# rlglab/minizero

Hardware: AMD Instinct MI355X
Metric: self-play leaf-evals/s (9x9 Go AlphaZero n=400) (higher is better)
Workload: dtype f32; 1 GPU; BASELINE configs[1]: 9x9 Go AlphaZero, n=400, 6 blocks x 64 ch, 256 parallel games per GPU, synthetic fixed-weight net (seed 0), Dirichlet noise + random rotation + softmax-count moves (reference defaults); games_per_gpu=256, actor_num_simulation=400, pipeline_lanes=1, backend=nccl

## Files before the change

minizero_amd/csrc/net_body.h:

```cpp
#pragma once
#include "net_dev.h"
#include <type_traits>

#ifndef MZ_HPROF
#define MZ_HPROF(k)
#endif

namespace mz {

struct TowerArgs {
    int nlayers, cin0, C, OT;
    int in_bits;
    int has_stem;
    unsigned w_off[48], b_off[48];
};

template <int H, int W>
struct TileMap {
    static constexpr int P = H * W, PW = W + 2;
    static constexpr int PT = (P + 15) / 16;
    static constexpr bool kCorner = (P % 16 == 1) && H > 1 && W > 1 && PT >= 2;
    static constexpr int VQ = kCorner ? W - 1 : -1;
    static constexpr int PT0 = (PT + 1) / 2, PT1 = PT - PT0;
    short q[PT * 16];
// ... 493 lines not shown
        const float acc = (FP && xlds && xpw != 0) ? dotChain<16, true, true>(xrd + xo, xstride, w, 1, C) : dotChain<16>(xrd + xo, xstride, w, 1, C);
        float v = acc + ((j < PC) ? hp.pconv_b[j] : hp.vconv_b[0]);
        v = v > 0.0f ? v : 0.0f;
        if (j < PC) { pf[i] = v; } else { vf[p] = v; }
    }
    __syncthreads();
    MZ_HPROF(6);

    for (int a = tid; a < A; a += NT) {
        const float v = (BIGA ? dotChain<64, true, true>(pf, 1, hp.pfc_wT + a, A, PC * P) : FP ? dotChain<16, true, true>(pf, 1, hp.pfc_wT + a, A, PC * P) : dotChain<16>(pf, 1, hp.pfc_wT + a, A, PC * P)) + hp.pfc_b[a];
        lg[a] = v;
        logit[size_t(b) * A + a] = v;
    }
    if (BIGA && NT == 512 && A <= 384) {
        if (tid >= 384) {
            for (int o = tid - 384; o < VH; o += 256) {
                const int o2 = o + 128 < VH ? o + 128 : o;
                const float* const xs2[2] = {vf, vf};
                const float* const ws2[2] = {hp.vfc1_wT + o, hp.vfc1_wT + o2};
                float acc2[2];
                dotChainK<32, 2, true, true>(xs2, 1, ws2, VH, P, acc2);
                const float v0 = acc2[0] + hp.vfc1_b[o], v1 = acc2[1] + hp.vfc1_b[o2];
                h1[o] = v0 > 0.0f ? v0 : 0.0f;
                if (o + 128 < VH) { h1[o2] = v1 > 0.0f ? v1 : 0.0f; }
            }
        }
    } else {
        const int vo = (NT >= 256 && A <= 128) ? 128 : 0;
        for (int o = (tid - vo + NT) % NT; o < VH; o += NT) {
            const float v = (FP ? dotChain<16, true, true>(vf, 1, hp.vfc1_wT + o, VH, P) : dotChain<16>(vf, 1, hp.vfc1_wT + o, VH, P)) + hp.vfc1_b[o];
            h1[o] = v > 0.0f ? v : 0.0f;
        }
    }
    __syncthreads();
    MZ_HPROF(7);

    if (tid == 64) {
        const float acc = BIGA ? dotChain<32, true, true>(h1, 1, hp.vfc2_w, 1, VH) : FP ? dotChain<16, true, true>(h1, 1, hp.vfc2_w, 1, VH) : dotChain<16>(h1, 1, hp.vfc2_w, 1, VH);
        value[b] = mz_tanhf(acc + hp.vfc2_b[0]);
    }
    if (wave == 0) {
        float m = -3.4e38f;
        for (int a = lane; a < A; a += 64) { m = lg[a] > m ? lg[a] : m; }
        for (int o = 32; o > 0; o >>= 1) { float m2 = __shfl_xor(m, o); m = m2 > m ? m2 : m; }
        for (int a = lane; a < A; a += 64) { lg[a] = mz_expf(lg[a] - m); }
        __builtin_amdgcn_wave_barrier();
        __builtin_amdgcn_fence(__ATOMIC_ACQ_REL, "wavefront");
        const float s = orderedSumWave(lg, A, lane);
        for (int a = lane; a < A; a += 64) { policy[size_t(b) * A + a] = lg[a] / s; }
        MZ_HPROF(8);
    }
}


}
```

minizero_amd/csrc/sim.hip:

```cpp
#include "sim_az_body.h"
#include "sim_mz_body.h"

namespace mz {

MZ_SPEC_WAYS_IS(16);

template <int H, int W, int CIN0_PAD, int CDYN_PAD, int CPAD>
__global__ __launch_bounds__(512) void sim_kernel_mz(const SimArgs* __restrict__ a_, int sim0, int nsims, int host_start, int pre_epoch)
{
    CSimArgs* a = (CSimArgs*)a_;
    extern __shared__ __attribute__((aligned(16))) float tiles[];
    const int g = blockIdx.x, tid = threadIdx.x, lane = tid & 63, wave = tid >> 6;
    constexpr int CM = CIN0_PAD > CDYN_PAD ? (CIN0_PAD > CPAD ? CIN0_PAD : CPAD) : (CDYN_PAD > CPAD ? CDYN_PAD : CPAD);
    constexpr int kTileFloats = kTowerTiles * CM * planeStride(H, W);
    double* rcp_w = reinterpret_cast<double*>(tiles + kTileFloats);
    const int rcp_n = a->rcp_n;
    for (int i = tid; i < rcp_n; i += 512) { rcp_w[i] = a->pv.rcp_tab[i]; }
    LdsCDouble* rcp_lds = (LdsCDouble*)rcp_w;
    const int tab_n = rcp_n - 2;
    double* sqrt_w = rcp_w + rcp_n;
    float* bias_w = reinterpret_cast<float*>(sqrt_w + tab_n);
    int* spec_w = reinterpret_cast<int*>(bias_w + tab_n + (tab_n & 1));
    for (int i = tid; i < tab_n; i += 512) { sqrt_w[i] = a->pv.sqrt_tab[i]; bias_w[i] = a->pv.bias_tab[i]; }
    if (!a->atari) {
// ... 455 lines not shown
#ifdef MZ_SIM_TPROF
    {
        unsigned long long h[64];
        if (hipMemcpyFromSymbol(h, HIP_SYMBOL(g_tp), sizeof(h)) == hipSuccess && h[63]) {
            fprintf(stderr, "[mz sim tprof] cycles per layer (game 0, avg over %llu towers):", h[63]);
            for (int i = 0; i < 14; ++i) { fprintf(stderr, " %.0f", double(h[i]) / double(h[63])); }
            fprintf(stderr, "\n");
        }
    }
#endif
    if (sim_prof_.n == 0) { return; }
    hipLaunchKernelGGL(sim_prof_fold, dim3(1), dim3(1), 0, stream_, sim_prof_.p + sim_prof_.n - kSimProfTail);
    if (hipStreamSynchronize(stream_) != hipSuccess) { return; }
    std::vector<unsigned long long> h(sim_prof_.n);
    if (hipMemcpy(h.data(), sim_prof_.p, h.size() * sizeof(unsigned long long), hipMemcpyDeviceToHost) != hipSuccess) { return; }
    const std::vector<unsigned long long> tail(h.end() - kSimProfTail, h.end());
    h.resize(h.size() - kSimProfTail);
    double skipped = 0, skipped_max = 0, sims_all = 0;
    for (size_t g = 0; g < h.size() / 8; ++g) {
        const double sk = double(h[g * 8 + 4] >> 32);
        h[g * 8 + 4] &= 0xFFFFFFFFull;
        skipped += sk; sims_all += double(h[g * 8 + 4]);
        skipped_max = std::max(skipped_max, sk / std::max(1.0, double(h[g * 8 + 4])));
    }
    { double ps = 0, ac = 0, kk = 0; for (size_t g = 0; g < h.size() / 8; ++g) { ps += double(h[g * 8 + 7] >> 40); ac += double((h[g * 8 + 7] >> 20) & 0xFFFFF); kk += double(h[g * 8 + 7] & 0xFFFFF); } fprintf(stderr, "[mz sim prof] path speculation: %.0f passes, %.0f levels taken, %.0f walks that found a remembered path\n", ps, ac, kk); }
    const char* names[4] = {"select+leaf", "tower", "heads", "cand+expand"};
    const size_t G = h.size() / 8;
    double tot_all = 0, tot_max = 0;
    for (int k = 0; k < 4; ++k) {
        double sum = 0, mx = 0, sims = 0;
        for (size_t g = 0; g < G; ++g) { sum += double(h[g * 8 + k]); mx = std::max(mx, double(h[g * 8 + k])); sims += double(h[g * 8 + 4]); }
        fprintf(stderr, "[mz sim prof] %-12s avg %8.2f us per simulation (slowest game %8.2f us)\n", names[k], sum / std::max(1.0, sims) * 0.01,
                mx / std::max(1.0, sims / G) * 0.01);
        tot_all += sum / std::max(1.0, sims) * 0.01;
    }
    {
        double sel = 0, lev = 0, sims = 0, maxlev = 0;
        double helped = 0;
        const unsigned long long low = (1ull << 40) - 1;
        for (size_t g = 0; g < G; ++g) { sel += double(h[g * 8 + 5]); lev += double(h[g * 8 + 6] & low); helped += double(h[g * 8 + 6] >> 40); sims += double(h[g * 8 + 4]); maxlev = std::max(maxlev, double(h[g * 8 + 6] & low) / std::max(1.0, double(h[g * 8 + 4]))); }
        fprintf(stderr, "[mz sim prof] levels taken over from the helper waves: %.0f (%.1f %% of all levels)\n", helped, 100.0 * helped / std::max(1.0, lev));
        fprintf(stderr, "[mz sim prof] select alone avg %8.2f us, path length avg %.2f (deepest game avg %.2f) -> %.2f us per level\n", sel / std::max(1.0, sims) * 0.01,
                lev / std::max(1.0, sims), maxlev, sel / std::max(1.0, lev) * 0.01);
    }
    for (size_t g = 0; g < G; ++g) { tot_max = std::max(tot_max, double(h[g * 8] + h[g * 8 + 1] + h[g * 8 + 2] + h[g * 8 + 3]) / std::max(1.0, double(h[g * 8 + 4])) * 0.01); }
    fprintf(stderr, "[mz sim prof] total        avg %8.2f us per simulation (slowest game %8.2f us)\n", tot_all, tot_max);
    {
        double tw = 0, hd = 0;
        for (size_t g = 0; g < G; ++g) { tw += double(h[g * 8 + 1]); hd += double(h[g * 8 + 2]); }
        const double ran = std::max(1.0, sims_all - skipped);
        fprintf(stderr, "[mz sim prof] terminal leaves: network skipped in %.0f of %.0f simulations (%.2f %%; the game with the most: %.2f %%) -> per simulation that ran them: tower %.2f us, heads %.2f us\n",
                skipped, sims_all, 100.0 * skipped / std::max(1.0, sims_all), 100.0 * skipped_max, tw / ran * 0.01, hd / ran * 0.01);
    }
    fprintf(stderr, "[mz sim prof] value first: %llu of %.0f simulations in the new order; %llu walks arrived at the previous simulation's leaf, %llu waited there (avg %.2f us); "
                    "%llu waits at the join in front of the leaf\n",
            tail[16], sims_all, tail[17], tail[18], double(tail[19]) / std::max(1.0, double(tail[18])) * 0.01, tail[20]);
    if (tail[8] > 0) {
        const double L = double(tail[8]), first = double(tail[9]) / L * 0.01, last = double(tail[10]) / L * 0.01, mean = double(tail[11]) / L * 0.01;
        const double helping = double(tail[12]) / L * 0.01;
        fprintf(stderr, "[mz sim prof] launches: %llu, avg per launch from the first game's start: first game done %.1f us, mean %.1f us, last %.1f us -> %.1f %% of the CU time idles at the end of a launch\n",
                tail[8], first, mean, last, 100.0 * (last - mean - helping) / std::max(1e-9, last));
        if (tail[13] > 0 || tail[15] > 0 || tail[21] > 0) {
            double tw = 0;
            for (size_t g = 0; g < G; ++g) { tw += double(h[g * 8 + 1]); }
            const double ran = sims_all - skipped, qn = double(tail[21]), qt = double(tail[22]), pn = double(tail[13]) + qn, pt = double(tail[14]) + qt;
            const double ln = double(tail[33]), lt = double(tail[34]);
            fprintf(stderr, "[mz sim prof] tail help: %.0f of the %.0f simulations that ran the network had a pair tower (%.2f %%): tower %.2f us with a helper, %.2f us alone; %llu games helped, "
                            "a CU helps for %.1f us per launch after its own game (%.1f %% of the launch)\n",
                    pn, ran, 100.0 * pn / std::max(1.0, ran), pt / std::max(1.0, pn) * 0.01, (tw - pt - lt) / std::max(1.0, ran - pn - ln) * 0.01, tail[15], helping,
                    100.0 * helping / std::max(1e-9, last));
            fprintf(stderr, "[mz sim prof] tail help, quad towers: %.0f of the %.0f simulations that ran the network had a quad tower (%.2f %%): tower %.2f us with three helpers, %.2f us with "
                            "one; %llu games went from pair to quad towers\n",
                    qn, ran, 100.0 * qn / std::max(1.0, ran), qt / std::max(1.0, qn) * 0.01, (pt - qt) / std::max(1.0, pn - qn) * 0.01, tail[23]);
            const double ia = double(tail[30]) / L * 0.01, ib = double(tail[31]) / L * 0.01, ic = double(tail[32]) / L * 0.01;
            fprintf(stderr, "[mz sim prof] tail help, idle CU time by the reason the CU stopped looking for a game to help (%% of the launch): (a) every running game of its XCD had its "
                            "helpers %.2f %%, (b) no game of its XCD was running any more %.2f %%, (c) only games with fewer than help_min_left simulations were left %.2f %%\n",
                    100.0 * ia / std::max(1e-9, last), 100.0 * ib / std::max(1e-9, last), 100.0 * ic / std::max(1e-9, last));
        }
        if (tail[33] > 0 || tail[35] > 0 || tail[36] > 0) {
            const double ran = sims_all - skipped, ln = double(tail[33]), taken = double(tail[35]);
            fprintf(stderr, "[mz sim prof] lending: %.0f of the %.0f simulations that ran the network had a tower lent by a game that was ahead (%.2f %%): tower %.2f us with the volunteer; "
                            "%llu offers taken, %llu of them withdrawn behind a terminal leaf, %llu taken too late; a volunteer waits %.2f us for its command and is away for %.2f us per "
                            "offer taken, %.1f us per launch and CU (%.1f %% of the launch)\n",
                    ln, ran, 100.0 * ln / std::max(1.0, ran), double(tail[34]) / std::max(1.0, ln) * 0.01, tail[35], tail[37], tail[36], double(tail[38]) / std::max(1.0, taken) * 0.01,
                    double(tail[39]) / std::max(1.0, taken) * 0.01, double(tail[39]) / std::max(1.0, double(G)) / L * 0.01, 100.0 * double(tail[39]) / std::max(1.0, double(G)) / L * 0.01 / std::max(1e-9, last));
        }
    }
}

static size_t simLdsBound(size_t tile_bytes, int n, int A, size_t head_floats)
{
    const size_t rcp_n = size_t(n) + 5, max_depth = size_t(n) + 3;
    return tile_bytes + rcp_n * (2 * sizeof(double) + sizeof(float)) + kSpecWords * sizeof(int) + (size_t(5) * (A + 1) + 26 + 18 * 12 + 2 * max_depth + 2 + head_floats) * sizeof(float) +
           size_t(kGoSeenCap) * sizeof(uint64_t);
}

int Net::uploadSimArgs(const SimArgs& a)
{
    static_assert(sizeof(SimArgs) % 4 == 0, "SimArgs is copied as words");
    if (sim_args_host_.size() != sizeof(SimArgs) || memcmp(sim_args_host_.data(), &a, sizeof(SimArgs)) != 0) {
        if (!sim_args_.ensure(sizeof(SimArgs))) { setError("hipMalloc of the simulation arguments failed"); return MZ_ERR_DEVICE; }
        MZ_HIP(hipStreamSynchronize(stream_));
        MZ_HIP(hipMemcpy(sim_args_.p, &a, sizeof(SimArgs), hipMemcpyHostToDevice));
        sim_args_host_.assign(reinterpret_cast<const char*>(&a), reinterpret_cast<const char*>(&a) + sizeof(SimArgs));
    }
    return MZ_OK;
// ... 64 lines not shown
    a.use_gumbel = gum ? 1 : 0;
    if (gum) { a.gum = *gum; }
    a.start = d_start;
    a.no_spec = getenv("MZ_NO_SPEC") ? atoi(getenv("MZ_NO_SPEC")) : 0;
    if (getenv("MZ_SIM_PROF")) {
        rc = simProfBuffer(gv.games, &a.prof);
        if (rc) { return rc; }
    }
    if (wide) {
        if (precision_ == 1) {
            if (!makeTowerArgsBf16(&a.tb)) { setError("simLaunch: bf16x3 tower not available for this network"); return MZ_OK; }
            a.wfrag = wfrag_.p;
        }
        size_t scratch = std::max(std::max(goLeafSmemBytes(gv, pool.v_.max_depth), azCandSmemBytes(gv.A)), gumbelSmemBytes(gv.A));
        scratch = std::max(scratch, size_t(2) * pool.v_.bound_cap * sizeof(float));
        int lf = 0;
        size_t lds = 0, tile_bytes = 0;
        if (!simWidePlan(gv.n, gv.kind, pool.v_.max_depth - 3, a.hp, gv.channels, gv.W32, goLeafSmemBytes(gv, pool.v_.max_depth), scratch, &lf, &lds, &tile_bytes)) { return MZ_OK; }
        a.cand_coop = (gv.A > kCandCoopMax && gv.A <= kCandCoopMaxW && candCoopSmemBytesW(gv.A, 8) <= tile_bytes) ? 2 : candCoopSmemBytes(gv.A, 8) <= tile_bytes ? 1 : 0;
        return simLaunchWide(a, gv, pool.v_.max_depth, d_rot, sim0, nsims, host_start, lf, lds, launched);
    }
    const int H = desc_.hidden_channel_height, W = desc_.hidden_channel_width, C = desc_.num_hidden_channels;
    const int cmax = c0 > C ? c0 : C;
    const bool bf = precision_ == 1;
    if (bf) {
        if (!makeTowerArgsBf16(&a.tb)) { setError("simLaunch: bf16x3 tower not available for this network"); return MZ_OK; }
        a.wfrag = wfrag_.p;
    }
    bool help = false;
    if (tail_help_ && !bf && !(a.no_spec & 32) && H == 9 && W == 9 && c0 == 20 && C == 64 && a.ta.OT == 4 && gv.n == 9 && gv.kind == kGo && gv.games >= 2 && gv.games <= cu_count_ &&
        gv.games <= kHpMaxGames && helpCmdUnits(gv.channels * gv.W32) <= kHpMaxUnits) {
        const int env_min = getenv("MZ_SIM_HELP_MIN") ? std::max(1, atoi(getenv("MZ_SIM_HELP_MIN"))) : 0;
        const size_t words = helpWords(C, H * W);
        if (!sim_help_mem_.ensure(size_t(gv.games) * words)) { setError("hipMalloc of the help blocks failed"); return MZ_ERR_DEVICE; }
        a.help = sim_help_mem_.p;
        a.help_words = static_cast<int>(words);
        a.help_min_left = env_min ? std::min(env_min, kSimHelpMinLeft) : kSimHelpMinLeft;
        a.lend_lead = getenv("MZ_SIM_LEND_LEAD") ? std::max(1, atoi(getenv("MZ_SIM_LEND_LEAD"))) : kSimLendLead;
        help = nsims >= (env_min ? env_min : kSimHelpMinLaunch);
        if (help) { MZ_HIP(hipMemsetAsync(sim_help_mem_.p, 0, size_t(gv.games) * words * sizeof(unsigned), stream_)); }
    }
    const int start_bits = (host_start ? 1 : 0) | (help ? 2 : 0);
    const size_t tile_bytes = bf ? size_t(4) * ((((H + 2) * (W + 2) + 16) / 16) * 16) * 128 + size_t(64) * planeStride(H, W) * 4
                                 : size_t(kTowerTiles) * cmax * planeStride(H, W) * sizeof(float);
    const size_t heads = (size_t(a.hp.PC) * a.hp.P + a.hp.P + a.hp.VH + a.hp.A + 16) * sizeof(float);
    size_t scratch = std::max(std::max(goLeafSmemBytes(gv, pool.v_.max_depth), azCandSmemBytes(gv.A)), gumbelSmemBytes(gv.A));
    scratch = std::max(scratch, size_t(2) * pool.v_.bound_cap * sizeof(float));
    a.cand_coop = candCoopSmemBytes(gv.A, 8) <= tile_bytes ? 1 : 0;
    if (scratch > tile_bytes || heads > tile_bytes / kTowerTiles) {
        setError("simLaunch: the tree phases need %zu B / the heads %zu B of scratch, the tower tiles have %zu B", scratch, heads, tile_bytes);
        return MZ_OK;
    }
    const bool two_per_cu = !bf && H * W <= 64 && tile_bytes <= size_t(76) * 1024;
    const size_t lds = tile_bytes + size_t(a.rcp_n) * sizeof(double) +
                       (two_per_cu ? 0 : size_t(a.rcp_n) * (sizeof(double) + sizeof(float)) + kSpecWords * sizeof(int)) + (simXchgWords(gv.A, gv.channels, gv.W32) + 2 + 2 * size_t(pool.v_.max_depth) + 2) * sizeof(float) +
                       ((gv.kind == kGo && !two_per_cu) ? size_t(kGoSeenCap) * sizeof(uint64_t) + ((goLeafSmemBytes(gv, pool.v_.max_depth) + 7) & ~size_t(7)) : 0);
    rc = uploadSimArgs(a);
    if (rc) { return rc; }
    if (lds > size_t(160) * 1024) { setError("simLaunch: %zu bytes of LDS needed", lds); return MZ_OK; }
    if (bf) {
        if (H == 9 && W == 9 && c0 == 20 && C == 64 && gv.n == 9 && gv.kind == kGo && gv.W == 2) { *launched = true; return launchSimT<9, 9, 20, 64, 2, true>(reinterpret_cast<const SimArgs*>(sim_args_.p), gv.games, d_rot, sim0, nsims, host_start ? 1 : 0, lds, stream_); }
        if (H == 8 && W == 8 && c0 == 4 && C == 64 && gv.n == 8 && gv.kind == kOthello) { *launched = true; return launchSimT<8, 8, 4, 64, kRulesOthello, true>(reinterpret_cast<const SimArgs*>(sim_args_.p), gv.games, d_rot, sim0, nsims, host_start ? 1 : 0, lds, stream_); }
        return MZ_OK;
    }
#define MZ_SIM_LAUNCH(h, w, cin0, cpad, cpl) \
    if (H == h && W == w && c0 == cin0 && C == cpad && gv.n == h && rulesArg(gv.kind, gv.n) == cpl) { *launched = true; return launchSimT<h, w, cin0, cpad, cpl>(reinterpret_cast<const SimArgs*>(sim_args_.p), gv.games, d_rot, sim0, nsims, start_bits, lds, stream_); }
    MZ_SIM_CASES(MZ_SIM_LAUNCH)
#undef MZ_SIM_LAUNCH
    if (isGameVariant(gv.kind) && simVariantKernel(H, W, c0, C, gv.n, rulesArg(gv.kind, gv.n), reinterpret_cast<const SimArgs*>(sim_args_.p), gv.games, d_rot, sim0, nsims, start_bits, lds, stream_, &rc)) {
        *launched = rc == MZ_OK;
        return rc;
    }
    return MZ_OK;
}

bool Net::hasPreBoard() const
{
    if (desc_.type != 1 || !use_fused_) { return false; }
    TowerArgs t1, t2;
    int c0 = 0, cd = 0;
    if (!makeTowerArgs(repr_, true, true, &t1, &c0) || !makeTowerArgs(dyn_, false, true, &t2, &cd)) { return false; }
    const int H = desc_.hidden_channel_height, W = desc_.hidden_channel_width, C = desc_.num_hidden_channels;
#define MZ_SIM_PRE_HAS_B(h, w, cin0, cdyn, cpad) \
    if (H == h && W == w && c0 == cin0 && cd == cdyn && C == cpad) { return true; }
    MZ_SIM_MZ_BOARD_PRE_CASES(MZ_SIM_PRE_HAS_B)
#undef MZ_SIM_PRE_HAS_B
    return false;
}

bool Net::hasSimKernelMz(int num_simulation) const
{
    if ((desc_.type != 1 && desc_.type != 2) || !use_fused_) { return false; }
    if (simMzWidePlan(num_simulation, nullptr, nullptr, nullptr, nullptr, nullptr)) { return true; }
    TowerArgs t1, t2;
    int c0 = 0, cd = 0;
    if (desc_.type == 2) { c0 = desc_.num_hidden_channels; }
    else if (!makeTowerArgs(repr_, true, true, &t1, &c0)) { return false; }
    if (!makeTowerArgs(dyn_, false, true, &t2, &cd)) { return false; }
    const int H = desc_.hidden_channel_height, W = desc_.hidden_channel_width, C = desc_.num_hidden_channels;
    {
        size_t head_floats = 0;
        if (desc_.type == 2) { AtariHeadParams hp; makeAtariHeadParams(&hp); head_floats = atariHeadsSmemFloats(hp); }
        else { head_floats = (gumbelSmemBytes(desc_.action_size) + 3) / 4; }
        const size_t tile_bytes = size_t(kTowerTiles) * std::max(std::max(c0, cd), C) * planeStride(H, W) * sizeof(float);
        if (simLdsBound(tile_bytes, num_simulation, desc_.action_size, head_floats) > size_t(160) * 1024) { return false; }
    }
#define MZ_SIM_MZ_HAS(h, w, cin0, cdyn, cpad) \
    if (H == h && W == w && c0 == cin0 && cd == cdyn && C == cpad) { return true; }
    MZ_SIM_MZ_CASES(MZ_SIM_MZ_HAS)
// ... 228 lines not shown
```

minizero_amd/csrc/sim_args.h:

```cpp
#pragma once
#include "net.h"
#include "net_body.h"
#include "net_bf16_body.h"
#include "net_atari_body.h"
#include "pool_body.h"
#include "go_body.h"
#include "gumbel_body.h"
#include <type_traits>

namespace mz {

struct SimArgs {
    PoolView pv;
    GoDevView gv;
    TowerArgs ta;
    HeadParams hp;
    const float* params;
    float* act;
    float* act2;
    float *policy, *logit, *value;
    int *cand_count, *cand_action, *cand_player;
    float *cand_policy, *cand_logit, *value_io, *reward_io;
    int* err;
    int rcp_n;
    TowerArgs ta_dyn;
    float* hidden;
    const unsigned* root_feat;
    const unsigned long long* root_legal;
    const int* root_turn;
    int slots, A, LW, num_players;
    const float* root_noise;
    float noise_eps;
    int noise_kind;
    int use_gumbel;
    GumbelView gum;
    int* start;
    int atari, action_planes;
    AtariHeadParams ahp;
    float* reward;
    int no_spec;
    int cand_coop;
    const uint4* wfrag;
    TowerArgsBf16 tb;
    unsigned* cluster;
    int cluster_words, oct_words;
    unsigned* cluster_oct;
    unsigned long long* prof;
    int* pre_key;
    float *pre_policy, *pre_logit;
    int* pre_action;
    float *pre_value, *pre_reward;
    unsigned* pre_stat;
    int alt_base;
    int help_min_left;
    unsigned* help;
    int help_words;
    int lend_lead;
};

typedef __attribute__((address_space(4))) const SimArgs CSimArgs;
template <class T>
__device__ __forceinline__ T ldc(__attribute__((address_space(4))) const T* p)
{
    static_assert(sizeof(T) % 4 == 0 && std::is_trivially_copyable<T>::value, "word-copied");
    typedef __attribute__((address_space(4))) const unsigned CU;
    CU* s = (CU*)p;
    unsigned w[sizeof(T) / 4];
#pragma unroll
    for (size_t i = 0; i < sizeof(T) / 4; ++i) { w[i] = s[i]; }
    T t;
    __builtin_memcpy(&t, w, sizeof(T));
    return t;
}

__device__ __forceinline__ PoolView simPathView(PoolView pv, int* lds_path, int g)
{
    const size_t off = size_t(g) * pv.max_depth;
    pv.path = lds_path - off;
    pv.path_action = lds_path + pv.max_depth - off;
    pv.path_len = lds_path + 2 * pv.max_depth - g;
    pv.num_nodes = lds_path + 2 * pv.max_depth + 1 - g;
    pv.host_path_len = nullptr;
    pv.host_path_action = nullptr;
    return pv;
}

template <class T>
__device__ __forceinline__ T* opaquePtr(T* p)
{
    asm volatile("" : "+v"(p));
    return p;
}
__device__ __forceinline__ PoolView simPathViewSafe(PoolView pv, int* lds_path, int g)
{
    pv = simPathView(pv, opaquePtr(lds_path), g);
    return pv;
}

bool simVariantKernel(int H, int W, int c0, int C, int board_n, int cpl, const SimArgs* d_args, int games, const uint8_t* d_rot, int sim0, int nsims, int host_start, size_t lds,
                      hipStream_t s, int* rc);

}
```

minizero_amd/csrc/sim_az_body.h:

```cpp
#pragma once
#include "net.h"
#ifdef MZ_SIM_TPROF
__device__ unsigned long long g_tp[64];
__shared__ unsigned long long s_tp_prev;
__shared__ int s_tp_idx;
#define MZ_TPROF(slot)                                                                         \
    do {                                                                                       \
        if ((slot) == 3 && threadIdx.x == 0 && blockIdx.x == 0) {                              \
            const unsigned long long t_ = clock64();                                           \
            g_tp[s_tp_idx & 63] += t_ - s_tp_prev; s_tp_prev = t_; ++s_tp_idx;                 \
        }                                                                                      \
    } while (0)
#endif
#ifdef MZ_SIM_HPROF
#ifndef MZ_HPROF_BLOCK
#define MZ_HPROF_BLOCK 0
#endif
__device__ unsigned long long g_hp[16];
__shared__ unsigned long long s_hp_prev;
#define MZ_HPROF(k)                                                                                   \
    do {                                                                                              \
        if (threadIdx.x == 0 && blockIdx.x == MZ_HPROF_BLOCK) {                                       \
            const unsigned long long t_ = wall_clock64();                                             \
            if ((k) > 0) { g_hp[(k)] += t_ - s_hp_prev; } else { g_hp[15] += 1; }                     \
// ... 355 lines not shown
__device__ __noinline__ void simApplyRootNoise(CSimArgs* __restrict__ a, int g, int lane)
{
    g = __builtin_amdgcn_readfirstlane(g);
    const PoolView v = ldc(&a->pv);
    const size_t base = size_t(g) * v.cap;
    const int nc = v.rec[base].num_children;
    const size_t fc = base + v.rec[base].first_child;
    const float eps = a->noise_eps;
    for (int i = lane; i < nc; i += 64) {
        const float nz = a->root_noise[size_t(g) * v.A + i];
        if (a->noise_kind == kNoiseDirichlet) { v.rec[fc + i].policy = (1 - eps) * v.rec[fc + i].policy + eps * nz; }
        else { v.logit[fc + i] = v.logit[fc + i] + nz; }
        v.noise[fc + i] = nz;
    }
    waveSync();
}

template <int WPE>
__device__ __noinline__ void simGumbelStart(CSimArgs* __restrict__ a, int slot, bool host_start, int g, int lane, float* tiles, int* state_lds = nullptr)
{
    g = __builtin_amdgcn_readfirstlane(g);
    slot = __builtin_amdgcn_readfirstlane(slot);
    if (host_start && slot >= 1) { return; }
    int st = 0;
    if (slot >= 1 && !host_start) {
        const PoolView pv = ldc(&a->pv);
        GumbelView gum = ldc(&a->gum);
        if (state_lds) { gum.state = state_lds - size_t(g) * (3 + kGumbelMaxSample); }
        st = gumbelStepBody(pv, gum, slot, g, lane, tiles);
    }
    if (lane == 0) { a->start[g] = st; }
    waveSync();
}

template <int WPE, bool BIGA = false, bool FP = BIGA>
__device__ __forceinline__ void simHeadsImpl(CSimArgs* __restrict__ a, int g, int tid, float* tiles, const float* xtile, int xcs, int xpw, float* xchg)
{
    g = __builtin_amdgcn_readfirstlane(g);
    xcs = __builtin_amdgcn_readfirstlane(xcs);
    xpw = __builtin_amdgcn_readfirstlane(xpw);
    MZ_HPROF(0);
    const HeadParams hp = ldc(&a->hp);
    const SimXchg x{hp.A + (hp.A & 1)};
    const size_t ga = size_t(g) * hp.A;
    headsBody<BIGA, FP>(nullptr, hp, xchg + x.policy() - ga, xchg + x.logit() - ga, xchg + x.scalars() - g, nullptr, nullptr, 0, g, tid, 512, tiles, xtile, xcs, xpw);
    MZ_HPROF(1);
}
template <int WPE, bool BIGA = false, bool FP = BIGA>
__device__ __noinline__ void simHeads(CSimArgs* __restrict__ a, int g, int tid, float* tiles, const float* xtile, int xcs, int xpw, float* xchg)
{
    simHeadsImpl<WPE, BIGA, FP>(a, g, tid, tiles, xtile, xcs, xpw, xchg);
}

__device__ __forceinline__ bool simLeafTerminal(CSimArgs* __restrict__ a, const float* xchg)
{
    if (a->no_spec & 16) { return false; }
    const int A = a->gv.A;
    const SimXchg x{A + (A & 1)};
    return __builtin_amdgcn_readfirstlane(reinterpret_cast<const int*>(xchg + x.scalars())[6]) != 0;
}

constexpr int kSimProfTail = 40;
__device__ __forceinline__ void simProfEnter(unsigned long long* tail)
{
    atomicMin(tail + 0, wall_clock64() - tail[4]);
}
__device__ __forceinline__ void simProfExit(unsigned long long* tail)
{
    const unsigned long long t = wall_clock64() - tail[4];
    atomicMin(tail + 1, t);
    atomicMax(tail + 2, t);
    atomicAdd(tail + 3, t);
    atomicAdd(tail + 5, 1ull);
}

template <int H, int W, int CIN0_PAD, int CPAD, bool BF = false>
constexpr int simWavesPerEu() { return (!BF && H * W <= 64 && kTowerTiles * (CIN0_PAD > CPAD ? CIN0_PAD : CPAD) * planeStride(H, W) * 4 <= 76 * 1024) ? 4 : 2; }
template <int H, int W, int CIN0_PAD, int CPAD, bool BF>
constexpr int simTileFloats() { return BF ? towerBf16LdsBytes<H, W>(true) / 4 : kTowerTiles * (CIN0_PAD > CPAD ? CIN0_PAD : CPAD) * planeStride(H, W); }

template <int H, int W, int CIN0_PAD, int CPAD>
__device__ __noinline__ const float* simTower(CSimArgs* __restrict__ a, int g, int tid, float* tiles, float* xchg)
{
    g = __builtin_amdgcn_readfirstlane(g);
#ifdef MZ_SIM_TPROF
    if (tid == 0 && g == 0) { s_tp_prev = clock64(); s_tp_idx = 0; g_tp[63] += 1; }
#endif
    g = __builtin_amdgcn_readfirstlane(g);
    const GoDevView gv = simLeafView(ldc(&a->gv), xchg, g);
    return towerBody<H, W, CIN0_PAD, CPAD>(reinterpret_cast<const float*>(gv.feat), a->params, *(const TowerArgs*)&a->ta, nullptr, g, tid, tiles);
}

template <int H, int W>
__device__ __noinline__ const float* simTowerBf16(CSimArgs* __restrict__ a, int g, int tid, float* tiles, float* xchg)
{
    g = __builtin_amdgcn_readfirstlane(g);
    const GoDevView gv = simLeafView(ldc(&a->gv), xchg, g);
    return towerBodyBf16<H, W>(reinterpret_cast<const unsigned*>(gv.feat), a->wfrag, a->params, *(const TowerArgsBf16*)&a->tb, nullptr, g, tid,
                               reinterpret_cast<char*>(tiles));
}

template <int H, int W, int CIN0_PAD, int CPAD, int MODE>
__device__ __forceinline__ const float* simTowerHelped(CSimArgs* __restrict__ a, int g, int tid, float* tiles, float* xchg, int seq, unsigned xseq, int* abort_lds, bool lent = false)
{
    g = __builtin_amdgcn_readfirstlane(g);
    seq = __builtin_amdgcn_readfirstlane(seq);
// ... 251 lines not shown
            if (!(st == 2 ? simHelpTower<H, W, CIN0_PAD, CPAD, kHpModeQuad>(a, cl - 1, slot, xseq, tid, tiles, bits, s_help)
                          : simHelpTower<H, W, CIN0_PAD, CPAD, kHpModePair>(a, cl - 1, 1, xseq, tid, tiles, bits, s_help))) { return; }
            __syncthreads();
        }
        __syncthreads();
    }
}

template <int H, int W, int CIN0_PAD, int CPAD, int CPL, bool BF = false>
__global__ __launch_bounds__(512) __attribute__((amdgpu_waves_per_eu(simWavesPerEu<H, W, CIN0_PAD, CPAD, BF>(), 4))) void sim_kernel(const SimArgs* __restrict__ a_, const uint8_t* __restrict__ rot_tab, int sim0, int nsims, int host_start)
{
    CSimArgs* a = (CSimArgs*)a_;
    extern __shared__ __attribute__((aligned(16))) float tiles[];
    const int g = blockIdx.x, tid = threadIdx.x, lane = tid & 63, wave = tid >> 6;
    const int games = gridDim.x;
    constexpr int WPE = simWavesPerEu<H, W, CIN0_PAD, CPAD, BF>();
    constexpr int kTileFloats = simTileFloats<H, W, CIN0_PAD, CPAD, BF>();
    double* rcp_w = reinterpret_cast<double*>(tiles + kTileFloats);
    for (int i = tid; i < a->rcp_n; i += 512) { rcp_w[i] = a->pv.rcp_tab[i]; }
    __syncthreads();
    LdsCDouble* rcp_lds = (LdsCDouble*)rcp_w;
    SpecMem spec{nullptr, nullptr, nullptr};
    int* spec_w = nullptr;
    const int path_words = 2 * a->pv.max_depth + 2;
    float* xchg = reinterpret_cast<float*>(rcp_w + a->rcp_n) + path_words;
    if constexpr (WPE == 2) {
        const int tab_n = a->rcp_n - 2;
        double* sqrt_w = rcp_w + a->rcp_n;
        float* bias_w = reinterpret_cast<float*>(sqrt_w + tab_n);
        spec_w = reinterpret_cast<int*>(bias_w + tab_n + (tab_n & 1));
        for (int i = tid; i < tab_n; i += 512) { sqrt_w[i] = a->pv.sqrt_tab[i]; bias_w[i] = a->pv.bias_tab[i]; }
        if (tid < kSpecWays) { spec_w[tid * kSpecWay] = 0; }
        if (tid < 8) { spec_w[kSpecWays * kSpecWay + tid] = 0; }
        if (tid < kHelpSegs) { spec_w[kSpecHelp + tid * kHelpSeg] = 0; }
        __syncthreads();
        spec = SpecMem{(a->no_spec & 1) ? nullptr : (LdsI32*)spec_w, (LdsCFloat*)bias_w, (LdsCDbl*)sqrt_w};
        xchg = reinterpret_cast<float*>(spec_w + kSpecWords) + path_words;
    }
    const uint64_t* seen_lds = nullptr;
    if constexpr (CPL > 0 && WPE == 2) {
        uint64_t* sw = reinterpret_cast<uint64_t*>(xchg + ((simXchgWordsDev(a->gv.A, a->gv.channels, a->gv.W32) + 1) & ~1));
        for (int i = tid; i < kGoSeenCap; i += 512) { sw[i] = a->gv.snap[g].seen[i]; }
        __syncthreads();
        seen_lds = sw;
    }
    uint64_t* leaf_smem = nullptr;
    if constexpr (CPL > 0 && WPE == 2) {
        const HeadParams hp = ldc(&a->hp);
        if (hp.VH <= 256 && (hp.PC + 1) * hp.P <= 384 && hp.A <= 384 && !(a->no_spec & 8)) {
            leaf_smem = const_cast<uint64_t*>(seen_lds) + kGoSeenCap;
            uint64_t* zk = leaf_smem + goLeafKeyWord(a->gv.Ppad, a->gv.W, a->pv.max_depth);
            for (int i = tid; i < 2 * a->gv.P; i += 512) { zk[i] = a->gv.key[i]; }
            __syncthreads();
        }
    }
    unsigned long long* prof = a->prof ? a->prof + size_t(g) * 8 : nullptr;
    int* const node_count = reinterpret_cast<int*>(xchg) - 1;
    if (tid == 0) { *node_count = a->pv.num_nodes[g]; }
    if (prof && tid == 0) { simProfEnter(a->prof + size_t(games) * 8); }
    constexpr bool kHelp = !BF && WPE == 2 && CPL > 0 && pairTowerShape<H, W, CPAD>();
    __shared__ int s_help[kHelp ? kVfWords : 4];
    const bool help_on = kHelp && (host_start & 2) != 0;
    unsigned* const help_blk = help_on ? a->help + size_t(g) * a->help_words : nullptr;
    unsigned help_xseq = 0;
    unsigned long long pair_n = 0, pair_t = 0;
    unsigned long long quad_n = 0, quad_t = 0;
    unsigned long long lent_n = 0, lent_t = 0;
    unsigned long long lend_t = 0;
    if (help_on && tid == 0) { s_help[0] = 0; s_help[1] = 0; hpStoreU(help_blk + kHpXcc, hpXccId()); }
    bool vf = false;
    if constexpr (kHelp) {
        vf = leaf_smem != nullptr && !a->use_gumbel && !a->pv.value_rescale && a->cand_coop != 2 && !(a->no_spec & 64);
        if (tid >= kVfBackup && tid < kVfWords) { s_help[tid] = 0; }
    }
    unsigned long long vf_t0 = 0, vf_n = 0;
    const bool lend_on = kHelp && help_on && vf && !(a->no_spec & 256);
    __syncthreads();
    for (int s = 0; s < nsims; ++s) {
        const int slot = sim0 + s;
        const int rot = rot_tab[size_t(s) * games + g];
        unsigned long long t0 = 0, t1 = 0, t2 = 0, t3 = 0, t4 = 0;
        if (prof) { t0 = (vf && s > 0) ? vf_t0 : wall_clock64(); }
        if (kHelp && vf) {
            if constexpr (kHelp) {
                if (wave == 0) {
                    if (s == 0) {
                        if (slot == 1 && a->root_noise) { simApplyRootNoise<WPE>(a, g, lane); }
                        simWalkVf(a, g, lane, rcp_lds, spec, xchg, (a->no_spec & 2) ? 0 : 1, -1, 0, s_help);
                        if (lend_on && lane == 0) { __hip_atomic_store((LdsI32*)s_help + kVfWalked, 1, __ATOMIC_RELAXED, __HIP_MEMORY_SCOPE_WORKGROUP); }
                    } else {
                        const bool waited = vfWait((LdsI32*)s_help + kVfExpand, s, a->err, lane);
                        if (prof && waited && lane == 0) { s_help[kVfStats + 3] += 1; }
                        if (help_on && lane == 0) { hpStoreU(help_blk + kHpProgress, unsigned(s)); }
                    }
                    simLeafVf<CPL>(a, rot, slot, g, lane, xchg, seen_lds, leaf_smem, s_help);
                } else if (s == 0 && wave <= kHelpSegs && spec.w && !(a->no_spec & 2)) {
                    simSelectHelper(a, g, lane, wave, 1, rcp_lds, spec);
                } else if (lend_on && wave == 7) {
                    simLendScan(a, g, lane, s, nsims, help_blk, s_help);
                } else if (help_on && tid == 7 * 64) {
                    s_help[1] = simHelpMode(help_blk);
                }
            }
        } else if (wave == 0) {
            if (slot == 1 && a->root_noise) { simApplyRootNoise<WPE>(a, g, lane); }
            if (a->use_gumbel) { simGumbelStart<WPE>(a, slot, s == 0 && (host_start & 1) != 0, g, lane, tiles); }
// ... 3 lines not shown
        } else if (kHelp && help_on && tid == 7 * 64) {
            s_help[1] = simHelpMode(help_blk);
        }
        __syncthreads();
        const int help_mode = (kHelp && help_on) ? __builtin_amdgcn_readfirstlane(s_help[1]) : 0;
        const bool lent = lend_on && __builtin_amdgcn_readfirstlane(s_help[kVfOffer]) != 0;
        const bool pair = help_mode == 1 || lent, quad = help_mode == 2;
        const bool term = simLeafTerminal(a, xchg);
        if constexpr (kHelp) {
            if (lend_on) {
                if (lent && term && tid == 7 * 64) { hpStoreU(help_blk + kHpOffer, 0u); }
                const int lend_to = __builtin_amdgcn_readfirstlane(s_help[kVfLend]);
                if (lend_to != 0) {
                    const unsigned long long tl0 = prof ? wall_clock64() : 0;
                    if (!simLendTower<H, W, CIN0_PAD, CPAD>(a, lend_to - 1, __builtin_amdgcn_readfirstlane(s_help[kVfLend + 1]), tid, tiles, s_help)) { return; }
                    if (prof) { const unsigned long long d = wall_clock64() - tl0; t0 += d; lend_t += d; }
                }
            }
        }
        if constexpr (CPL > 0) {
            if (!term) {
                simLeafPlanes<CPL>(a, rot, g, wave, lane, leaf_smem ? leaf_smem : reinterpret_cast<const uint64_t*>(tiles), xchg);
                __syncthreads();
            }
        }
        if (prof) { t1 = wall_clock64(); }
        const float* xt = nullptr;
        if (!term) {
            if constexpr (BF) { xt = simTowerBf16<H, W>(a, g, tid, tiles, xchg); }
            else if constexpr (WPE == 4) {
                const GoDevView gvt = simLeafView(ldc(&a->gv), xchg, g);
                xt = towerBody<H, W, CIN0_PAD, CPAD>(reinterpret_cast<const float*>(gvt.feat), a->params, *(const TowerArgs*)&a->ta, nullptr, g, tid, tiles);
            }
            else if constexpr (kHelp) {
                if (pair) {
                    xt = simTowerPair<H, W, CIN0_PAD, CPAD>(a, g, tid, tiles, xchg, s + 1, help_xseq, s_help, lent ? 1 : 0);
                    if (!xt) { return; }
                    help_xseq += unsigned(a->ta.nlayers);
                    if (lent && tid == 7 * 64) { hpStoreU(help_blk + kHpOffer, 0u); }
                }
                else if (quad) {
                    xt = simTowerQuad<H, W, CIN0_PAD, CPAD>(a, g, tid, tiles, xchg, s + 1, help_xseq, s_help);
                    if (!xt) { return; }
                    help_xseq += unsigned(a->ta.nlayers);
                }
                else { xt = simTower<H, W, CIN0_PAD, CPAD>(a, g, tid, tiles, xchg); }
            }
            else { xt = simTower<H, W, CIN0_PAD, CPAD>(a, g, tid, tiles, xchg); }
        }
        __syncthreads();
        if (prof) { t2 = wall_clock64(); }
        if constexpr (WPE == 4) { if (!term) { simHeadsImpl<WPE>(a, g, tid, tiles, xt, planeStride(H, W), W + 2, xchg); } }
        else if (leaf_smem && wave >= 6) { simLeafRest<CPL>(a, rot, slot, g, lane, xchg, seen_lds, leaf_smem, 7 - wave); }
        else if (!term) { simHeads<WPE, false, (MZ_HEADS_FP != 0)>(a, g, tid, tiles, xt, planeStride(H, W), W + 2, xchg); }
        else if (leaf_smem) { __syncthreads(); __syncthreads(); }
        __syncthreads();
        if (prof) { t3 = wall_clock64(); }
        if (kHelp && vf) {
            if constexpr (kHelp) {
                const bool more = s + 1 < nsims;
                if (wave == 0) {
                    simBackupOnly<WPE>(a, slot, g, lane, tiles, xchg);
                    vfPublish((LdsI32*)s_help + kVfBackup, s + 1, lane);
                    if (prof && tid == 0) {
                        t4 = wall_clock64();
                        prof[0] += t1 - t0 + (term ? t3 - t1 : 0); prof[1] += term ? 0 : t2 - t1; prof[2] += term ? 0 : t3 - t2; prof[3] += t4 - t3;
                        prof[4] += 1 + (static_cast<unsigned long long>(term) << 32);
                        if (pair && !lent && !term) { pair_n += 1; pair_t += t2 - t1; }
                        if (quad && !term) { quad_n += 1; quad_t += t2 - t1; }
                        if (lent && !term) { lent_n += 1; lent_t += t2 - t1; }
                        vf_n += 1;
                    }
                    vf_t0 = t4;
                    if (more) {
                        if (slot + 1 == 1 && a->root_noise) {
                            vfWait((LdsI32*)s_help + kVfExpand, s + 1, a->err, lane);
                            simApplyRootNoise<WPE>(a, g, lane);
                        }
                        simWalkVf(a, g, lane, rcp_lds, spec, xchg, (a->no_spec & 2) ? 0 : s + 2, __builtin_amdgcn_readfirstlane(s_help[kVfLeaf]), s + 1, s_help);
                        if (lend_on && lane == 0) { __hip_atomic_store((LdsI32*)s_help + kVfWalked, s + 2, __ATOMIC_RELAXED, __HIP_MEMORY_SCOPE_WORKGROUP); }
                    }
                } else if (wave <= kHelpSegs) {
                    if (more && spec.w && !(a->no_spec & 2)) {
                        vfWait((LdsI32*)s_help + kVfBackup, s + 1, a->err, lane);
                        simSelectHelper(a, g, lane, wave, s + 2, rcp_lds, spec);
                    }
                } else {
                    simCandPipeVf<WPE>(a, rot, slot, g, lane, wave - 4, s + 1, tiles, xchg, s_help);
                }
            }
            continue;
        }
        if (wave == 0) { simCandGather<WPE>(a, rot, g, lane, tiles, xchg); }
        __syncthreads();
        {
            const int A = a->gv.A;
            const SimXchg x{A + (A & 1)};
            if (a->cand_coop) { simCandRank(A, reinterpret_cast<const int*>(xchg + x.scalars())[1], wave, lane, tiles); }
        }
        __syncthreads();
        {
            const bool split = !a->pv.value_rescale;
            if (wave == 0) { simCandExpand<WPE>(a, rot, slot, g, lane, tiles, xchg, split ? 1 : 0); }
            else if (wave == 1 && split) { simBackupOnly<WPE>(a, slot, g, lane, tiles, xchg); }
        }
        __syncthreads();
        if (prof && tid == 0) {
            t4 = wall_clock64();
            prof[0] += t1 - t0 + (term ? t3 - t1 : 0); prof[1] += term ? 0 : t2 - t1; prof[2] += term ? 0 : t3 - t2; prof[3] += t4 - t3;
            prof[4] += 1 + (static_cast<unsigned long long>(term) << 32);
            if (pair && !term) { pair_n += 1; pair_t += t2 - t1; }
            if (quad && !term) { quad_n += 1; quad_t += t2 - t1; }
        }
        if (kHelp && help_on && tid == 0) { hpStoreU(help_blk + kHpProgress, unsigned(s) + 1u); }
    }
    if constexpr (kHelp) {
        if (vf) {
            __syncthreads();
            if (help_on && tid == 0) { hpStoreU(help_blk + kHpProgress, unsigned(nsims)); }
            if (prof && tid == 0) {
                unsigned long long* ptail = a->prof + size_t(games) * 8;
                atomicAdd(ptail + 16, vf_n);
                for (int i = 0; i < 4; ++i) { atomicAdd(ptail + 17 + i, static_cast<unsigned long long>(s_help[kVfStats + i])); }
                if (lend_on) {
                    atomicAdd(ptail + 33, lent_n); atomicAdd(ptail + 34, lent_t);
                    for (int i = 0; i < 4; ++i) { atomicAdd(ptail + 35 + i, static_cast<unsigned long long>(s_help[kVfLendStat + i])); }
                    atomicAdd(ptail + 39, lend_t);
                }
            }
        }
    }
    if (tid == 0) { a->pv.num_nodes[g] = *node_count; }
    if (prof && tid == 0) {
        simProfExit(a->prof + size_t(games) * 8);
        if (pair_n) { atomicAdd(a->prof + size_t(games) * 8 + 13, pair_n); atomicAdd(a->prof + size_t(games) * 8 + 14, pair_t); }
        if (quad_n) { atomicAdd(a->prof + size_t(games) * 8 + 21, quad_n); atomicAdd(a->prof + size_t(games) * 8 + 22, quad_t); atomicAdd(a->prof + size_t(games) * 8 + 23, pair_n ? 1ull : 0ull); }
    }
    if (prof && tid == 0 && spec_w) {
        prof[7] += (static_cast<unsigned long long>(spec_w[kSpecWays * kSpecWay + 1]) << 40) | (static_cast<unsigned long long>(spec_w[kSpecWays * kSpecWay + 5]) << 20) | spec_w[kSpecWays * kSpecWay + 3];
        prof[6] += static_cast<unsigned long long>(spec_w[kSpecWays * kSpecWay + 7]) << 40;
    }
    if constexpr (kHelp) {
        if (help_on) {
            const int A = a->gv.A;
            const SimXchg x{A + (A & 1)};
            __syncthreads();
            simHelpTail<H, W, CIN0_PAD, CPAD>(a, g, tid, tiles, reinterpret_cast<unsigned*>(xchg + x.feat()), nsims, s_help);
        }
    }
}


}
```

Measured before the change: 1.734 million leaf-evals/s.

## Add shape-specialized 9x9 heads path with LDS-staged weights and prefetched FC operands

Adds a heads implementation specialized to the 9x9 Go, 64-channel shape. It stages the small head weights and biases into LDS once per launch, and makes the policy-FC and value-FC1 waves load their weight columns into registers before the 1x1 convolutions run. The FC loops then use double-buffered LDS loads with the next weight group refilled behind the FMAs, to hide global-memory latency in the per-simulation heads. It uses extra LDS and many registers, which could lower occupancy or spill, and it can be turned off with an environment variable or a no_spec bit.

```diff
diff --git a/minizero_amd/csrc/net_body.h b/minizero_amd/csrc/net_body.h
--- a/minizero_amd/csrc/net_body.h
+++ b/minizero_amd/csrc/net_body.h
@@ -569,5 +569,194 @@
     }
 }
 
-
-}
+struct HeadsAhead {
+    static constexpr int C = 64, P = 81, N = 9, A = 82, PC = 2, VH = 256;
+    static constexpr int kPconvW = 0, kVconvW = 128, kConvB = 192, kFc2W = 196, kFc2B = 452, kPfcB = 456, kFc1B = 540, kWords = 796;
+    static constexpr int kPf = 0, kVf = 164, kH1 = 248, kLg = 504, kScratch = 504 + 82 + 16;
+    static constexpr int kRows = 81, kGroup = 27;
+    __host__ __device__ static bool shape(const HeadParams& hp) { return hp.C == C && hp.P == P && hp.A == A && hp.PC == PC && hp.VH == VH; }
+};
+
+__device__ __forceinline__ void headsAheadStage(const HeadParams& hp, float* __restrict__ hw, int tid, int NT)
+{
+    typedef HeadsAhead L;
+    for (int i = tid; i < L::PC * L::C; i += NT) { hw[L::kPconvW + i] = hp.pconv_w[i]; }
+    for (int i = tid; i < L::C; i += NT) { hw[L::kVconvW + i] = hp.vconv_w[i]; }
+    for (int i = tid; i < 4; i += NT) { hw[L::kConvB + i] = i < L::PC ? hp.pconv_b[i] : i == L::PC ? hp.vconv_b[0] : 0.0f; }
+    for (int i = tid; i < L::VH; i += NT) { hw[L::kFc2W + i] = hp.vfc2_w[i]; }
+    for (int i = tid; i < 4; i += NT) { hw[L::kFc2B + i] = i == 0 ? hp.vfc2_b[0] : 0.0f; }
+    for (int i = tid; i < L::kFc1B - L::kPfcB; i += NT) { hw[L::kPfcB + i] = i < L::A ? hp.pfc_b[i] : 0.0f; }
+    for (int i = tid; i < L::VH; i += NT) { hw[L::kFc1B + i] = hp.vfc1_b[i]; }
+}
+
+template <int I0, int I1, int GQ, class WF, class PRE>
+__device__ __forceinline__ void aheadChain(float& acc, __attribute__((address_space(3))) const float* x, WF wf, PRE pre)
+{
+    typedef float vf4 __attribute__((ext_vector_type(4)));
+    typedef __attribute__((address_space(3))) const vf4 LF4;
+    constexpr int Q0 = I0 / 4, NQ = (I1 + 3) / 4 - Q0, NG = (NQ + GQ - 1) / GQ;
+    vf4 xb[2][GQ];
+#pragma unroll
+    for (int k = 0; k < GQ; ++k) { if (k < NQ) { xb[0][k] = *(LF4*)(x + 4 * (Q0 + k)); } }
+#pragma unroll
+    for (int g = 0; g < NG; ++g) {
+        pre(g);
+#pragma unroll
+        for (int k = 0; k < GQ; ++k) { if ((g + 1) * GQ + k < NQ) { xb[(g + 1) & 1][k] = *(LF4*)(x + 4 * (Q0 + (g + 1) * GQ + k)); } }
+        __builtin_amdgcn_sched_barrier(0);
+#pragma unroll
+        for (int k = 0; k < GQ; ++k) {
+#pragma unroll
+            for (int e = 0; e < 4; ++e) {
+                const int i = 4 * (Q0 + g * GQ + k) + e;
+                if (i >= I0 && i < I1) { acc = __builtin_fmaf(xb[g & 1][k][e], wf(i), acc); }
+            }
+        }
+        __builtin_amdgcn_sched_barrier(0);
+    }
+}
+
+template <int CS, int PW>
+__device__ __forceinline__ void headsBodyAhead(const HeadParams& hp, float* __restrict__ policy_, float* __restrict__ logit_, float* __restrict__ value_, int tid,
+                                               float* __restrict__ sm, const float* __restrict__ xlds, const float* __restrict__ hw_)
+{
+    typedef HeadsAhead L;
+    typedef float vf4 __attribute__((ext_vector_type(4)));
+    typedef __attribute__((address_space(3))) const float LF;
+    typedef __attribute__((address_space(3))) float LFW;
+    typedef __attribute__((address_space(3))) const vf4 LF4;
+    typedef __attribute__((address_space(1))) const float GF;
+    static_assert((L::C - 1) * CS * 4 + (L::N + 1) * PW * 4 < 65536, "the conv1x1 reads its x operand at immediate offsets");
+    LF* hw = (LF*)hw_;
+    LF* xt = (LF*)xlds;
+    LFW* s = (LFW*)sm;
+    const int lane = tid & 63, wave = tid >> 6;
+
+    MZ_HPROF(5);
+    constexpr int R = L::kRows, G = L::kGroup;
+    const bool pol = wave < 2;
+    const int a = tid < L::A ? tid : L::A - 1, o = (tid - 128) & (L::VH - 1);
+    GF* wcol = pol ? (GF*)hp.pfc_wT + a : (GF*)hp.vfc1_wT + o;
+    int wstride = __builtin_amdgcn_readfirstlane(pol ? L::A : L::VH);
+    int wnext = __builtin_amdgcn_readfirstlane(pol ? R : 0);
+    int wstride2 = __builtin_amdgcn_readfirstlane(pol ? L::A : 0);
+    int xrow = pol ? L::kPf : L::kVf, brow = pol ? L::kPfcB + a : L::kFc1B + o;
+    asm volatile("" : "+v"(wcol), "+s"(wstride), "+s"(wnext), "+s"(wstride2), "+v"(xrow), "+v"(brow));
+    float w[R];
+    if (wave < 6) {
+#pragma unroll
+        for (int k = 0; k < R; ++k) { w[k] = wcol[k * wstride]; }
+    }
+    __builtin_amdgcn_sched_barrier(0);
+
+    if (tid < (L::PC + 1) * L::P) {
+        const int j = tid / L::P, p = tid - j * L::P;
+        LF* xp = xt + (p / L::N + 1) * PW + p % L::N + 1;
+        LF* wj = hw + (j < L::PC ? L::kPconvW + j * L::C : L::kVconvW);
+        float acc = 0.0f;
+        constexpr int CG = 16;
+        float xv[2][CG];
+        vf4 wq[2][CG / 4];
+#pragma unroll
+        for (int k = 0; k < CG; ++k) { xv[0][k] = xp[k * CS]; }
+#pragma unroll
+        for (int k = 0; k < CG / 4; ++k) { wq[0][k] = *(LF4*)(wj + 4 * k); }
+#pragma unroll
+        for (int g = 0; g < L::C / CG; ++g) {
+            if (g + 1 < L::C / CG) {
+#pragma unroll
+                for (int k = 0; k < CG; ++k) { xv[(g + 1) & 1][k] = xp[((g + 1) * CG + k) * CS]; }
+#pragma unroll
+                for (int k = 0; k < CG / 4; ++k) { wq[(g + 1) & 1][k] = *(LF4*)(wj + (g + 1) * CG + 4 * k); }
+            }
+            __builtin_amdgcn_sched_barrier(0);
+#pragma unroll
+            for (int k = 0; k < CG; ++k) { acc = __builtin_fmaf(xv[g & 1][k], wq[g & 1][k / 4][k & 3], acc); }
+            __builtin_amdgcn_sched_barrier(0);
+        }
+        float v = acc + hw[L::kConvB + j];
+        v = v > 0.0f ? v : 0.0f;
+        s[j < L::PC ? L::kPf + tid : L::kVf + p] = v;
+    }
+    __syncthreads();
+    MZ_HPROF(6);
+
+    if (wave < 6) {
+        constexpr int GQ = 5;
+        static_assert(R == 3 * G && L::PC * L::P == 2 * R && L::P == R, "three groups at the entry, three behind them");
+        static_assert(2 * 4 * GQ >= G && 3 * 4 * GQ >= 2 * G, "a group of w is refilled behind the fmas that read it");
+        float w3[G];
+        float acc = 0.0f;
+        GF* wn = wcol + wnext * wstride;
+        aheadChain<0, R, GQ>(acc, s + xrow, [&](int i) { return w[i]; },
+            [&](int g) {
+                if (g == 0) {
+#pragma unroll
+                    for (int k = 0; k < G; ++k) { w3[k] = wn[k * wstride2]; }
+                }
+                if (g == 2) {
+#pragma unroll
+                    for (int k = 0; k < G; ++k) { w[k] = wn[(G + k) * wstride2]; }
+                }
+                if (g == 3) {
+#pragma unroll
+                    for (int k = 0; k < G; ++k) { w[G + k] = wn[(2 * G + k) * wstride2]; }
+                }
+            });
+        if (pol) {
+            aheadChain<R, 2 * R, GQ>(acc, s + L::kPf, [&](int i) { return i < R + G ? w3[i - R] : w[i - R - G]; }, [](int) {});
+        }
+        const float v = acc + hw[brow];
+        if (pol) {
+            if (tid < L::A) {
+                s[L::kLg + tid] = v;
+                logit_[tid] = v;
+            }
+        } else {
+            s[L::kH1 + o] = v > 0.0f ? v : 0.0f;
+        }
+    }
+    __syncthreads();
+    MZ_HPROF(7);
+
+    if (tid == 64) {
+        float acc = 0.0f;
+        constexpr int GQ = 4;
+        vf4 hb[2][GQ], wb[2][GQ];
+#pragma unroll
+        for (int k = 0; k < GQ; ++k) { hb[0][k] = *(LF4*)(s + L::kH1 + 4 * k); wb[0][k] = *(LF4*)(hw + L::kFc2W + 4 * k); }
+#pragma unroll
+        for (int g = 0; g < L::VH / (4 * GQ); ++g) {
+            if (g + 1 < L::VH / (4 * GQ)) {
+#pragma unroll
+                for (int k = 0; k < GQ; ++k) {
+                    hb[(g + 1) & 1][k] = *(LF4*)(s + L::kH1 + 4 * ((g + 1) * GQ + k));
+                    wb[(g + 1) & 1][k] = *(LF4*)(hw + L::kFc2W + 4 * ((g + 1) * GQ + k));
+                }
+            }
+            __builtin_amdgcn_sched_barrier(0);
+#pragma unroll
+            for (int k = 0; k < GQ; ++k) {
+#pragma unroll
+                for (int e = 0; e < 4; ++e) { acc = __builtin_fmaf(hb[g & 1][k][e], wb[g & 1][k][e], acc); }
+            }
+            __builtin_amdgcn_sched_barrier(0);
+        }
+        value_[0] = mz_tanhf(acc + hw[L::kFc2B]);
+    }
+    if (wave == 0) {
+        float* lg = sm + L::kLg;
+        float m = -3.4e38f;
+        for (int i = lane; i < L::A; i += 64) { m = lg[i] > m ? lg[i] : m; }
+        for (int o = 32; o > 0; o >>= 1) { float m2 = __shfl_xor(m, o); m = m2 > m ? m2 : m; }
+        for (int i = lane; i < L::A; i += 64) { lg[i] = mz_expf(lg[i] - m); }
+        __builtin_amdgcn_wave_barrier();
+        __builtin_amdgcn_fence(__ATOMIC_ACQ_REL, "wavefront");
+        const float sum = orderedSumWave(lg, L::A, lane);
+        for (int i = lane; i < L::A; i += 64) { policy_[i] = lg[i] / sum; }
+        MZ_HPROF(8);
+    }
+}
+
+
+}
diff --git a/minizero_amd/csrc/sim.hip b/minizero_amd/csrc/sim.hip
--- a/minizero_amd/csrc/sim.hip
+++ b/minizero_amd/csrc/sim.hip
@@ -531,6 +531,8 @@
         fprintf(stderr, "[mz sim prof] terminal leaves: network skipped in %.0f of %.0f simulations (%.2f %%; the game with the most: %.2f %%) -> per simulation that ran them: tower %.2f us, heads %.2f us\n",
                 skipped, sims_all, 100.0 * skipped / std::max(1.0, sims_all), 100.0 * skipped_max, tw / ran * 0.01, hd / ran * 0.01);
     }
+    fprintf(stderr, "[mz sim prof] heads ahead: %llu of the %.0f simulations that ran the network used the heads with their operands delivered ahead\n", tail[7],
+            sims_all - skipped);
     fprintf(stderr, "[mz sim prof] value first: %llu of %.0f simulations in the new order; %llu walks arrived at the previous simulation's leaf, %llu waited there (avg %.2f us); "
                     "%llu waits at the join in front of the leaf\n",
             tail[16], sims_all, tail[17], tail[18], double(tail[19]) / std::max(1.0, double(tail[18])) * 0.01, tail[20]);
@@ -701,9 +703,17 @@
         return MZ_OK;
     }
     const bool two_per_cu = !bf && H * W <= 64 && tile_bytes <= size_t(76) * 1024;
-    const size_t lds = tile_bytes + size_t(a.rcp_n) * sizeof(double) +
+    size_t lds = tile_bytes + size_t(a.rcp_n) * sizeof(double) +
                        (two_per_cu ? 0 : size_t(a.rcp_n) * (sizeof(double) + sizeof(float)) + kSpecWords * sizeof(int)) + (simXchgWords(gv.A, gv.channels, gv.W32) + 2 + 2 * size_t(pool.v_.max_depth) + 2) * sizeof(float) +
                        ((gv.kind == kGo && !two_per_cu) ? size_t(kGoSeenCap) * sizeof(uint64_t) + ((goLeafSmemBytes(gv, pool.v_.max_depth) + 7) & ~size_t(7)) : 0);
+    if (!bf && !two_per_cu && H == 9 && W == 9 && c0 == 20 && C == 64 && gv.n == 9 && rulesArg(gv.kind, gv.n) == 2 && HeadsAhead::shape(a.hp) &&
+        !(getenv("MZ_SIM_HEADS_LDS") && atoi(getenv("MZ_SIM_HEADS_LDS")) == 0)) {
+        const size_t off = (lds + 15) & ~size_t(15), end = off + HeadsAhead::kWords * sizeof(float);
+        if (end + kVfWords * sizeof(int) <= size_t(160) * 1024 && HeadsAhead::kScratch * sizeof(float) <= tile_bytes / kTowerTiles) {
+            a.heads_lds = static_cast<int>(off / sizeof(float));
+            lds = end;
+        }
+    }
     rc = uploadSimArgs(a);
     if (rc) { return rc; }
     if (lds > size_t(160) * 1024) { setError("simLaunch: %zu bytes of LDS needed", lds); return MZ_OK; }
diff --git a/minizero_amd/csrc/sim_args.h b/minizero_amd/csrc/sim_args.h
--- a/minizero_amd/csrc/sim_args.h
+++ b/minizero_amd/csrc/sim_args.h
@@ -56,6 +56,7 @@
     unsigned* help;
     int help_words;
     int lend_lead;
+    int heads_lds;
 };
 
 typedef __attribute__((address_space(4))) const SimArgs CSimArgs;
diff --git a/minizero_amd/csrc/sim_az_body.h b/minizero_amd/csrc/sim_az_body.h
--- a/minizero_amd/csrc/sim_az_body.h
+++ b/minizero_amd/csrc/sim_az_body.h
@@ -431,6 +431,16 @@
     simHeadsImpl<WPE, BIGA, FP>(a, g, tid, tiles, xtile, xcs, xpw, xchg);
 }
 
+template <int H, int W>
+__device__ __forceinline__ void simHeadsAhead(CSimArgs* __restrict__ a, int tid, float* tiles, const float* xtile, float* xchg, const float* hw)
+{
+    MZ_HPROF(0);
+    const HeadParams hp = ldc(&a->hp);
+    const SimXchg x{HeadsAhead::A + (HeadsAhead::A & 1)};
+    headsBodyAhead<planeStride(H, W), W + 2>(hp, xchg + x.policy(), xchg + x.logit(), xchg + x.scalars(), tid, tiles, xtile, hw);
+    MZ_HPROF(1);
+}
+
 __device__ __forceinline__ bool simLeafTerminal(CSimArgs* __restrict__ a, const float* xchg)
 {
     if (a->no_spec & 16) { return false; }
@@ -788,6 +798,16 @@
             uint64_t* zk = leaf_smem + goLeafKeyWord(a->gv.Ppad, a->gv.W, a->pv.max_depth);
             for (int i = tid; i < 2 * a->gv.P; i += 512) { zk[i] = a->gv.key[i]; }
             __syncthreads();
+        }
+    }
+    constexpr bool kAhead = !BF && H == 9 && W == 9 && CIN0_PAD == 20 && CPAD == 64 && CPL == 2;
+    [[maybe_unused]] const float* heads_w = nullptr;
+    [[maybe_unused]] unsigned long long ahead_n = 0;
+    if constexpr (kAhead) {
+        const int off = a->heads_lds;
+        if (off > 0) {
+            headsAheadStage(ldc(&a->hp), tiles + off, tid, 512);
+            if (!(a->no_spec & 512)) { heads_w = tiles + off; }
         }
     }
     unsigned long long* prof = a->prof ? a->prof + size_t(g) * 8 : nullptr;
@@ -897,7 +917,12 @@
         if (prof) { t2 = wall_clock64(); }
         if constexpr (WPE == 4) { if (!term) { simHeadsImpl<WPE>(a, g, tid, tiles, xt, planeStride(H, W), W + 2, xchg); } }
         else if (leaf_smem && wave >= 6) { simLeafRest<CPL>(a, rot, slot, g, lane, xchg, seen_lds, leaf_smem, 7 - wave); }
-        else if (!term) { simHeads<WPE, false, (MZ_HEADS_FP != 0)>(a, g, tid, tiles, xt, planeStride(H, W), W + 2, xchg); }
+        else if (!term) {
+            bool ahead = false;
+            if constexpr (kAhead) { ahead = heads_w != nullptr; }
+            if (ahead) { if constexpr (kAhead) { simHeadsAhead<H, W>(a, tid, tiles, xt, xchg, heads_w); } }
+            else { simHeads<WPE, false, (MZ_HEADS_FP != 0)>(a, g, tid, tiles, xt, planeStride(H, W), W + 2, xchg); }
+        }
         else if (leaf_smem) { __syncthreads(); __syncthreads(); }
         __syncthreads();
         if (prof) { t3 = wall_clock64(); }
@@ -914,6 +939,7 @@
                         if (pair && !lent && !term) { pair_n += 1; pair_t += t2 - t1; }
                         if (quad && !term) { quad_n += 1; quad_t += t2 - t1; }
                         if (lent && !term) { lent_n += 1; lent_t += t2 - t1; }
+                        if constexpr (kAhead) { if (heads_w && !term) { ahead_n += 1; } }
                         vf_n += 1;
                     }
                     vf_t0 = t4;
@@ -956,6 +982,7 @@
             prof[4] += 1 + (static_cast<unsigned long long>(term) << 32);
             if (pair && !term) { pair_n += 1; pair_t += t2 - t1; }
             if (quad && !term) { quad_n += 1; quad_t += t2 - t1; }
+            if constexpr (kAhead) { if (heads_w && !term) { ahead_n += 1; } }
         }
         if (kHelp && help_on && tid == 0) { hpStoreU(help_blk + kHpProgress, unsigned(s) + 1u); }
     }
@@ -978,6 +1005,7 @@
     if (tid == 0) { a->pv.num_nodes[g] = *node_count; }
     if (prof && tid == 0) {
         simProfExit(a->prof + size_t(games) * 8);
+        if constexpr (kAhead) { if (ahead_n) { atomicAdd(a->prof + size_t(games) * 8 + 7, ahead_n); } }
         if (pair_n) { atomicAdd(a->prof + size_t(games) * 8 + 13, pair_n); atomicAdd(a->prof + size_t(games) * 8 + 14, pair_t); }
         if (quad_n) { atomicAdd(a->prof + size_t(games) * 8 + 21, quad_n); atomicAdd(a->prof + size_t(games) * 8 + 22, quad_t); atomicAdd(a->prof + size_t(games) * 8 + 23, pair_n ? 1ull : 0ull); }
     }
```

After: 1.760 million leaf-evals/s (median of 6 runs). 1.5% higher.
